# PKU-VCL-Geometry/GeoSplatting

Measured on AMD Instinct MI355X. Metric: fwd+bwd views/sec at 2M Gaussians, 800x800, higher is better.
Workload: dtype f32

## Files before the change

geosplatting_amd/csrc/gs_cube.h:

```cpp
#pragma once
#include "gs_common.h"

struct FaceMap { int a, b, c; float sx, sy; };
__device__ __forceinline__ FaceMap face_map(int s)
{
    const int axis = s >> 1;
    FaceMap m;
    m.a = axis == 0 ? 2 : 0;
    m.b = axis == 1 ? 2 : 1;
    m.c = axis;
    m.sx = (s == 0 || s == 5) ? -1.0f : 1.0f;
    m.sy = s == 2 ? 1.0f : -1.0f;
    return m;
}

__device__ __forceinline__ int select_face(const float* d)
{
    const float ax = fabsf(d[0]), ay = fabsf(d[1]), az = fabsf(d[2]);
    int f; float c;
    if (az > fmaxf(ax, ay)) { f = 4; c = d[2]; }
    else if (ay > ax)       { f = 2; c = d[1]; }
    else                    { f = 0; c = d[0]; }
    return f + (c < 0.0f ? 1 : 0);
}
// ... 102 lines not shown
    for (int i = 0; i < 4; ++i) { ok[i] = valid && fp.idx[i] >= 0; safe[i] = ok[i] ? fp.idx[i] : 0; }
    float t[4][3];
#pragma unroll
    for (int i = 0; i < 4; ++i) {
        const float* p = tex + (size_t)safe[i] * 3;
        t[i][0] = p[0]; t[i][1] = p[1]; t[i][2] = p[2];
    }
    bool has_miss = false;
#pragma unroll
    for (int i = 0; i < 4; ++i) {
        if (!ok[i]) { t[i][0] = t[i][1] = t[i][2] = 0.0f; }
        has_miss = has_miss || (valid && fp.idx[i] < 0);
    }
    if (has_miss) {
#pragma unroll
        for (int c = 0; c < 3; ++c) {
            const float s = (t[0][c] + t[1][c] + t[2][c] + t[3][c]) / 3.0f;
#pragma unroll
            for (int i = 0; i < 4; ++i) if (fp.idx[i] < 0) t[i][c] = s;
        }
    }
    if (!valid) {
        out[0] = out[1] = out[2] = 0.0f;
        if (WITH_GRAD) { for (int i = 0; i < 9; ++i) dd[i] = 0.0f; }
        return;
    }
    const FaceMap m = face_map(fp.face);
    const float sgn_c = comp3(d, m.c) < 0.0f ? -1.0f : 1.0f;
#pragma unroll
    for (int c = 0; c < 3; ++c) {
        const float top = t[0][c] + fp.fx * (t[1][c] - t[0][c]);
        const float bot = t[2][c] + fp.fx * (t[3][c] - t[2][c]);
        out[c] = top + fp.fy * (bot - top);
        if (WITH_GRAD) {
            const float dtx = (t[1][c] - t[0][c]) + fp.fy * ((t[3][c] - t[2][c]) - (t[1][c] - t[0][c]));
            const float dty = bot - top;
            const float gx = dtx * 0.5f * (float)R, gy = dty * 0.5f * (float)R;
            float g[3] = { 0.0f, 0.0f, 0.0f };
            const float va = gx * m.sx * fp.inv_c, vb = gy * m.sy * fp.inv_c;
            const float vc = -(gx * fp.xn + gy * fp.yn) * fp.inv_c * sgn_c;
#pragma unroll
            for (int k = 0; k < 3; ++k) g[k] = (k == m.a ? va : 0.0f) + (k == m.b ? vb : 0.0f) + (k == m.c ? vc : 0.0f);
            dd[c * 3 + 0] = g[0]; dd[c * 3 + 1] = g[1]; dd[c * 3 + 2] = g[2];
        }
    }
}

template <bool XCD_LOCAL>
__device__ __forceinline__ void gs_add_scoped(float* p, float v)
{
    if (XCD_LOCAL) gs_atomic_add_xcd(p, v); else gs_atomic_add(p, v);
}

template <bool XCD_LOCAL>
__device__ __forceinline__ void wave_commit6_lds(float* stage, float* pa, float* pb, const float (&v)[6])
{
    const int lane = (int)(threadIdx.x & 63);
    unsigned long long* sp = reinterpret_cast<unsigned long long*>(stage);
    float* sv = stage + 256;
    __builtin_amdgcn_wave_barrier();
    sp[lane] = (unsigned long long)pa; sp[64 + lane] = (unsigned long long)pb;
#pragma unroll
    for (int c = 0; c < 6; ++c) sv[c * 64 + lane] = v[c];
    __builtin_amdgcn_fence(__ATOMIC_RELEASE, "wavefront");
    __builtin_amdgcn_wave_barrier();
    __builtin_amdgcn_fence(__ATOMIC_ACQUIRE, "wavefront");
#pragma unroll
    for (int k = 0; k < 6; ++k) {
        const int q = 64 * k + lane;
        const int src = q / 6, ch = q - 6 * src;
        const bool second = ch >= 3;
        float* base = (float*)sp[(second ? 64 : 0) + src];
        const float val = sv[ch * 64 + src];
        if (base != nullptr) gs_add_scoped<XCD_LOCAL>(base + (second ? ch - 3 : ch), val);
    }
}

template <bool XCD_LOCAL>
__device__ __forceinline__ void wave_add6(float* pa, float* pb, const float (&v)[6], float* stage)
{
    float* enda = nullptr; float* endb = nullptr;
    float pv[6] = { 0.f, 0.f, 0.f, 0.f, 0.f, 0.f };
    if (pa != nullptr || pb != nullptr) {
        enda = pa; endb = pb;
#pragma unroll
        for (int c = 0; c < 6; ++c) pv[c] = v[c];
    }
    wave_commit6_lds<XCD_LOCAL>(stage, enda, endb, pv);
}

template <bool XCD_LOCAL>
__device__ __forceinline__ void cube_scatter_wave(float* grad_tex, const CubeFp& fp, const float* g, float scale, bool valid,
                                                  float* stage)
{
#pragma unroll
    for (int row = 0; row < 2; ++row) {
        float* p[2]; float v[6];
#pragma unroll
        for (int j = 0; j < 2; ++j) {
            const int i = 2 * row + j;
            const bool on = valid && fp.valid && fp.idx[i] >= 0 && grad_tex != nullptr;
            const float w = on ? scale * fp.w[i] : 0.0f;
            p[j] = on ? grad_tex + (size_t)fp.idx[i] * 3 : nullptr;
            v[3 * j] = g[0] * w; v[3 * j + 1] = g[1] * w; v[3 * j + 2] = g[2] * w;
        }
        wave_add6<XCD_LOCAL>(p[0], p[1], v, stage);
    }
}

__device__ __forceinline__ void wave_commit6_lds_tagged(float* stage, float* pa, float* pb, const float (&v)[6])
{
    const int lane = (int)(threadIdx.x & 63);
    unsigned long long* sp = reinterpret_cast<unsigned long long*>(stage);
    float* sv = stage + 256;
    const bool act = pa != nullptr || pb != nullptr;
    const unsigned long long am = __ballot(act);
    if (am == 0ull) return;
    const int n6 = 6 * __popcll(am);
    const int rank = __popcll(am & ((1ull << lane) - 1ull));
    __builtin_amdgcn_wave_barrier();
    if (act) {
        sp[rank] = (unsigned long long)pa; sp[64 + rank] = (unsigned long long)pb;
#pragma unroll
        for (int c = 0; c < 6; ++c) sv[c * 64 + rank] = v[c];
    }
    __builtin_amdgcn_fence(__ATOMIC_RELEASE, "wavefront");
    __builtin_amdgcn_wave_barrier();
    __builtin_amdgcn_fence(__ATOMIC_ACQUIRE, "wavefront");
    for (int k = 0; 64 * k < n6; ++k) {
        const int q = 64 * k + lane;
        if (q < n6) {
            const int src = q / 6, ch = q - 6 * src;
            const bool second = ch >= 3;
            const unsigned long long tagged = sp[(second ? 64 : 0) + src];
            float* base = (float*)(tagged & ~1ull);
            const float val = sv[ch * 64 + src];
            if (base != nullptr) {
                float* dst = base + (second ? ch - 3 : ch);
                if (tagged & 1ull) gs_atomic_add_xcd(dst, val); else gs_atomic_add(dst, val);
            }
        }
    }
}

__device__ __forceinline__ void cube_scatter_wave_tagged(float* grad_tex, bool local, const CubeFp& fp, const float* g, float scale, bool valid,
                                                         float* stage)
{
#pragma unroll
    for (int row = 0; row < 2; ++row) {
        float* p[2]; float v[6];
#pragma unroll
        for (int j = 0; j < 2; ++j) {
            const int i = 2 * row + j;
            const bool on = valid && fp.valid && fp.idx[i] >= 0 && grad_tex != nullptr;
            const float w = on ? scale * fp.w[i] : 0.0f;
            p[j] = on ? (float*)((unsigned long long)(grad_tex + (size_t)fp.idx[i] * 3) | (local ? 1ull : 0ull)) : nullptr;
            v[3 * j] = g[0] * w; v[3 * j + 1] = g[1] * w; v[3 * j + 2] = g[2] * w;
        }
        wave_commit6_lds_tagged(stage, p[0], p[1], v);
    }
}
```

geosplatting_amd/csrc/gs_front.hip:

```cpp
#include "gs_common.h"
#include <string.h>
#pragma clang fp contract(off)
#include "gs_project_dev.h"
#include "gs_shade_dev.h"

template <int CTRL, int ROW_MASK>
__device__ __forceinline__ unsigned dpp_max_u32(unsigned v)
{
    const unsigned o = (unsigned)__builtin_amdgcn_update_dpp(0, (int)v, CTRL, ROW_MASK, 0xf, false);
    return o > v ? o : v;
}
__device__ __forceinline__ unsigned wave_max_u32_lane63(unsigned v)
{
    v = dpp_max_u32<0xB1, 0xf>(v);
    v = dpp_max_u32<0x4E, 0xf>(v);
    v = dpp_max_u32<0x141, 0xf>(v);
    v = dpp_max_u32<0x140, 0xf>(v);
    v = dpp_max_u32<0x142, 0xa>(v);
    v = dpp_max_u32<0x143, 0xc>(v);
    return v;
}

#define GS_FRONT_BLOCK 256
#define GS_FRONT_ITEMS 2
// ... 465 lines not shown
    int W, H;
};
struct TailViewsDev { TailViewDev v[GS_TAIL_MAX_VIEWS]; int n; };

#define GS_TAILP_BLOCK 1024
struct TailViewLds {
    unsigned long long vis, v_packed, packed_index;
    float cam[16];
    float cam_pos[3];
    float Wf, Hf;
    float pad;
};

struct TailLevelLds { unsigned long long tex, gtex; long long priv_off; int R, lds_off; };

template <int VPG>
__device__ __forceinline__ float tail_group_sum(float v)
{
    if (VPG >= 2) v = gs_dpp_add<0xB1, 0xf, 0xf>(v);
    if (VPG >= 4) v = gs_dpp_add<0x4E, 0xf, 0xf>(v);
    if (VPG >= 8) v = gs_dpp_add<0x141, 0xf, 0xf>(v);
    return v;
}

template <int BLOCK, int VPG>
__global__ void __launch_bounds__(BLOCK)
tail_proj_pairs_kernel(int N, TailViewsDev views, const float* __restrict__ means, const float* __restrict__ quats,
                       const float* __restrict__ scales, const float* __restrict__ opacities, float eps2d, int rec_stride,
                       float* __restrict__ v_means, float* __restrict__ v_quats, float* __restrict__ v_scales,
                       float* __restrict__ v_opacities, int accumulate)
{
    __shared__ TailViewLds s_views[VPG];
#pragma unroll
    for (int k = 0; k < VPG; ++k) {
        if ((int)threadIdx.x == k) {
            const TailViewDev& h = views.v[k];
            TailViewLds& d = s_views[k];
            d.vis = (unsigned long long)h.vis; d.v_packed = (unsigned long long)h.v_packed; d.packed_index = (unsigned long long)h.packed_index;
            const GsCam c = load_cam(h.viewmat, h.K);
#pragma unroll
            for (int i = 0; i < 9; ++i) d.cam[i] = c.R[i];
            d.cam[9] = c.t[0]; d.cam[10] = c.t[1]; d.cam[11] = c.t[2];
            d.cam[12] = c.fx; d.cam[13] = c.fy; d.cam[14] = c.cx; d.cam[15] = c.cy;
            d.cam_pos[0] = d.cam_pos[1] = d.cam_pos[2] = 0.0f;
            d.Wf = (float)h.W; d.Hf = (float)h.H; d.pad = 0.0f;
        }
    }
    __syncthreads();
    constexpr int G = BLOCK / VPG;
    const int view = (int)threadIdx.x & (VPG - 1), gl = (int)threadIdx.x / VPG;
    const TailViewLds& vw = s_views[view];
    const int n = (int)blockIdx.x * G + gl;
    const bool live = n < N && view < views.n;
    const int slot = live ? reinterpret_cast<const int32_t*>(vw.packed_index)[n] : -1;
    ProjGrad pg;
#pragma unroll
    for (int c = 0; c < 3; ++c) { pg.mean[c] = 0.0f; pg.scale[c] = 0.0f; }
#pragma unroll
    for (int c = 0; c < 4; ++c) pg.quat[c] = 0.0f;
    pg.op = 0.0f;
    if (slot >= 0) {
        const float* vp = reinterpret_cast<const float*>(vw.v_packed) + (size_t)slot * rec_stride;
        const float4 g0 = reinterpret_cast<const float4*>(vp)[0];
        const float2 g1 = reinterpret_cast<const float2*>(vp)[2];
        if (g0.x != 0.0f || g0.y != 0.0f || g0.z != 0.0f || g0.w != 0.0f || g1.x != 0.0f || g1.y != 0.0f) {
            const float4* vis = reinterpret_cast<const float4*>(vw.vis);
            const float4 r0 = vis[4 * (size_t)slot], r1 = vis[4 * (size_t)slot + 1], r3 = vis[4 * (size_t)slot + 3];
            const float mean[3] = { means[3 * (size_t)n], means[3 * (size_t)n + 1], means[3 * (size_t)n + 2] };
            const float scale[3] = { scales[3 * (size_t)n], scales[3 * (size_t)n + 1], scales[3 * (size_t)n + 2] };
            const float4 q4 = *reinterpret_cast<const float4*>(quats + 4 * (size_t)n);
            const float opac = opacities[n];
            GsCam cam;
#pragma unroll
            for (int i = 0; i < 9; ++i) cam.R[i] = vw.cam[i];
            cam.t[0] = vw.cam[9]; cam.t[1] = vw.cam[10]; cam.t[2] = vw.cam[11];
            cam.fx = vw.cam[12]; cam.fy = vw.cam[13]; cam.cx = vw.cam[14]; cam.cy = vw.cam[15];
            project_bwd_one(cam, mean, q4, scale, opac, vw.Wf, vw.Hf, eps2d, 2.0f * r0.z, r0.w, 2.0f * r1.x, r3.x,
                            g0.x, g0.y, g0.z, g0.w, g1.x, g1.y, 0.0f, pg);
        }
    }
#pragma unroll
    for (int c = 0; c < 3; ++c) { pg.mean[c] = tail_group_sum<VPG>(pg.mean[c]); pg.scale[c] = tail_group_sum<VPG>(pg.scale[c]); }
#pragma unroll
    for (int c = 0; c < 4; ++c) pg.quat[c] = tail_group_sum<VPG>(pg.quat[c]);
    pg.op = tail_group_sum<VPG>(pg.op);
    if (n < N) {
        if (view == 0 % VPG) {
#pragma unroll
            for (int c = 0; c < 3; ++c) v_means[3 * (size_t)n + c] += pg.mean[c];
        }
        if (view == 1 % VPG) {
            float4 q = accumulate ? *reinterpret_cast<float4*>(v_quats + 4 * (size_t)n) : make_float4(0.f, 0.f, 0.f, 0.f);
            q.x += pg.quat[0]; q.y += pg.quat[1]; q.z += pg.quat[2]; q.w += pg.quat[3];
            *reinterpret_cast<float4*>(v_quats + 4 * (size_t)n) = q;
        }
        if (view == 2 % VPG) {
#pragma unroll
            for (int c = 0; c < 3; ++c) v_scales[3 * (size_t)n + c] = (accumulate ? v_scales[3 * (size_t)n + c] : 0.0f) + pg.scale[c];
        }
        if (view == 3 % VPG) v_opacities[n] = (accumulate ? v_opacities[n] : 0.0f) + pg.op;
    }
}

template <int BLOCK, int VPG, bool DIFFUSE>
__global__ void __launch_bounds__(BLOCK)
tail_shade_pairs_kernel(int N, TailViewsDev views, const float* __restrict__ means, const float* __restrict__ normals,
                        const float* __restrict__ kd, const float* __restrict__ ks, float min_roughness, float max_metallic, EnvDev env,
                        int rec_stride, float* __restrict__ v_means, float* __restrict__ v_normals, float* __restrict__ v_kd,
                        float* __restrict__ v_ks, EnvGradDev eg, int accumulate, int mode_rt)
{
    const int mode = DIFFUSE ? GS_MODE_DIFFUSE : mode_rt;
    __builtin_assume(DIFFUSE || mode != GS_MODE_DIFFUSE);
    extern __shared__ __attribute__((aligned(16))) float s_grad[];
    __shared__ TailViewLds s_views[VPG];
    __shared__ TailLevelLds s_levels[GS_MAX_LEVELS];
    for (int i = threadIdx.x; i < eg.lds_floats; i += blockDim.x) s_grad[i] = 0.0f;
#pragma unroll
    for (int l = 0; l < GS_MAX_LEVELS; ++l) {
        if ((int)threadIdx.x == 64 + l) {
            TailLevelLds& d = s_levels[l];
            if (DIFFUSE) { d.tex = (unsigned long long)env.base; d.gtex = (unsigned long long)eg.base; d.priv_off = -1; d.R = env.base_res; d.lds_off = eg.lds_base; }
            else { d.tex = (unsigned long long)env.levels[l]; d.gtex = (unsigned long long)eg.levels[l]; d.priv_off = eg.priv ? eg.priv_level[l] : -1; d.R = env.res[l]; d.lds_off = eg.lds_level[l]; }
        }
    }
#pragma unroll
    for (int k = 0; k < VPG; ++k) {
        if ((int)threadIdx.x == k) {
            const TailViewDev& h = views.v[k];
            TailViewLds& d = s_views[k];
            d.vis = (unsigned long long)h.vis; d.v_packed = (unsigned long long)h.v_packed; d.packed_index = (unsigned long long)h.packed_index;
            const GsCam c = load_cam(h.viewmat, h.K);
#pragma unroll
            for (int i = 0; i < 9; ++i) d.cam[i] = c.R[i];
            d.cam[9] = c.t[0]; d.cam[10] = c.t[1]; d.cam[11] = c.t[2];
            d.cam[12] = c.fx; d.cam[13] = c.fy; d.cam[14] = c.cx; d.cam[15] = c.cy;
            d.cam_pos[0] = h.cam_pos[0]; d.cam_pos[1] = h.cam_pos[1]; d.cam_pos[2] = h.cam_pos[2];
            d.Wf = (float)h.W; d.Hf = (float)h.H; d.pad = 0.0f;
        }
    }
    __syncthreads();
    float* const stage = s_grad + eg.stage_off + (threadIdx.x >> 6) * 640;
    float* const priv = eg.priv ? eg.priv + (long long)gs_xcc_id() * eg.priv_stride : nullptr;
    constexpr int G = BLOCK / VPG;
    const int view = (int)threadIdx.x & (VPG - 1), gl = (int)threadIdx.x / VPG;
    const bool view_on = view < views.n;
    const TailViewLds& vw = s_views[view];
    const int stride = (int)gridDim.x * G;
    const int n_iter = (N + stride - 1) / stride;
    for (int it = 0; it < n_iter; ++it) {
        const int n = it * stride + (int)blockIdx.x * G + gl;
        const bool live = n < N && view_on;
        const int slot = live ? reinterpret_cast<const int32_t*>(vw.packed_index)[n] : -1;
        float mean[3] = { 0, 0, 0 }, normal[3] = { 0, 0, 0 }, kdn[3] = { 0, 0, 0 }, ksn[2] = { 0, 0 };
        if (live) {
            mean[0] = means[3 * (size_t)n]; mean[1] = means[3 * (size_t)n + 1]; mean[2] = means[3 * (size_t)n + 2];
            normal[0] = normals[3 * (size_t)n]; normal[1] = normals[3 * (size_t)n + 1]; normal[2] = normals[3 * (size_t)n + 2];
            kdn[0] = kd[3 * (size_t)n]; kdn[1] = kd[3 * (size_t)n + 1]; kdn[2] = kd[3 * (size_t)n + 2];
            const float2 ks2 = *reinterpret_cast<const float2*>(ks + 2 * (size_t)n);
            ksn[0] = ks2.x; ksn[1] = ks2.y;
        }
        float a_mean[3] = { 0, 0, 0 }, a_n[3] = { 0, 0, 0 }, a_kd[3] = { 0, 0, 0 }, a_ks[2] = { 0, 0 };
        const float* vp = reinterpret_cast<const float*>(vw.v_packed) + (size_t)(slot >= 0 ? slot : 0) * rec_stride;
        bool work = false;
        PairPre pre;
        float g[3] = { 0, 0, 0 };
        if (slot >= 0) {
            g[0] = vp[6]; g[1] = vp[7]; g[2] = vp[8];
            if (g[0] != 0.0f || g[1] != 0.0f || g[2] != 0.0f) {
                const float cp[3] = { vw.cam_pos[0], vw.cam_pos[1], vw.cam_pos[2] };
                shade_pair_pre(mean, normal, kdn, ksn, cp, min_roughness, max_metallic, mode, env, g, pre);
                work = true;
            }
        }
        float o_acc[3] = { 0, 0, 0 }, vd_acc[3] = { 0, 0, 0 }, v_mip = 0.0f;
#pragma unroll 1
        for (int lv = 0; lv < (DIFFUSE ? 1 : 2); ++lv) {
            const int l = work ? (lv == 0 ? pre.l0 : pre.l1) : -1;
            const bool on = l >= 0;
            const TailLevelLds& lt = s_levels[on ? l : 0];
            const float w = lv == 0 ? (pre.l1 < 0 ? 1.0f : 1.0f - pre.f) : pre.f;
            CubeFp fp;
            fp.valid = false;
            if (on) {
                float o[3], sv, dd[3];
                cube_fetch_vjp(reinterpret_cast<const float*>(lt.tex), lt.R, pre.dir, pre.v, o, sv, dd, fp);
#pragma unroll
                for (int c = 0; c < 3; ++c) { o_acc[c] = fmaf(w, o[c], o_acc[c]); vd_acc[c] = fmaf(w, dd[c], vd_acc[c]); }
                v_mip += lv == 0 ? -sv : sv;
            }
            const bool in_lds = on && lt.lds_off >= 0;
            if (in_lds) cube_scatter_lds(s_grad + lt.lds_off, fp, pre.v, w);
            const bool glob = on && !in_lds;
            const bool loc = glob && priv != nullptr && lt.priv_off >= 0;
            cube_scatter_wave_tagged(glob ? (loc ? priv + lt.priv_off : reinterpret_cast<float*>(lt.gtex)) : nullptr, loc, fp, pre.v, w, glob, stage);
        }
        if (work) shade_pair_post(pre, normal, kdn, g, mode, min_roughness, max_metallic, o_acc, vd_acc, v_mip, a_mean, a_n, a_kd, a_ks);
#pragma unroll
        for (int c = 0; c < 3; ++c) {
            a_mean[c] = tail_group_sum<VPG>(a_mean[c]); a_n[c] = tail_group_sum<VPG>(a_n[c]); a_kd[c] = tail_group_sum<VPG>(a_kd[c]);
        }
        a_ks[0] = tail_group_sum<VPG>(a_ks[0]); a_ks[1] = tail_group_sum<VPG>(a_ks[1]);
        if (n < N) {
            if (view == 0 % VPG) {
#pragma unroll
                for (int c = 0; c < 3; ++c) v_means[3 * (size_t)n + c] = (accumulate ? v_means[3 * (size_t)n + c] : 0.0f) + a_mean[c];
            }
            if (view == 1 % VPG) {
                float2 o = accumulate ? *reinterpret_cast<float2*>(v_ks + 2 * (size_t)n) : make_float2(0.f, 0.f);
                o.x += a_ks[0]; o.y += a_ks[1];
                *reinterpret_cast<float2*>(v_ks + 2 * (size_t)n) = o;
            }
            if (view == 2 % VPG) {
#pragma unroll
                for (int c = 0; c < 3; ++c) v_normals[3 * (size_t)n + c] = (accumulate ? v_normals[3 * (size_t)n + c] : 0.0f) + a_n[c];
            }
            if (view == 3 % VPG) {
#pragma unroll
                for (int c = 0; c < 3; ++c) v_kd[3 * (size_t)n + c] = (accumulate ? v_kd[3 * (size_t)n + c] : 0.0f) + a_kd[c];
            }
        }
    }
    __syncthreads();
    if (eg.lds_base >= 0) {
        const int cnt = 18 * env.base_res * env.base_res;
        for (int i = threadIdx.x; i < cnt; i += blockDim.x) {
            const float x = s_grad[eg.lds_base + i];
            if (x != 0.0f) gs_atomic_add(eg.base + i, x);
        }
    }
    for (int l = 0; l < env.L; ++l) {
        if (eg.lds_level[l] < 0) continue;
        const int cnt = 18 * env.res[l] * env.res[l];
        for (int i = threadIdx.x; i < cnt; i += blockDim.x) {
            const float x = s_grad[eg.lds_level[l] + i];
            if (x != 0.0f) gs_atomic_add(eg.levels[l] + i, x);
        }
    }
}

extern "C" int gs_tail_bwd_multi_parts(int parts, int N, int n_views, const GsTailView* views, const float* means, const float* quats,
                                       const float* scales, const float* opacities, const float* normals, const float* kd, const float* ks,
                                       float min_roughness, float max_metallic, int mode, const GsEnv* env, float eps2d, int rec_stride,
                                       float* v_means, float* v_quats, float* v_scales, float* v_opacities, float* v_normals, float* v_kd,
                                       float* v_ks, int accumulate, const GsEnvGrad* env_grad, void* priv_ws, size_t priv_ws_bytes, void* stream)
{
    GS_CHECK_ARG(parts >= 1 && parts <= 7 && (parts & 3) != 0, "parts: bit 0 = shading backward, bit 1 = projection backward, bit 2 = background launch");
    GS_CHECK_ARG(N >= 0 && n_views >= 1 && mode >= 0 && mode <= 2 && rec_stride >= 12 && (rec_stride % 4) == 0, "bad sizes, mode or record stride");
    GS_CHECK_ARG(views != nullptr && env_grad != nullptr, "null argument");
    EnvDev e;
    GS_CHECK_ARG(env_to_dev(env, e) == 0, "bad GsEnv");
    EnvGradDev eg;
    { const int rc = env_grad_to_dev(__func__, env_grad, e, mode, eg); if (rc != GS_OK) return rc; }
    ShadeBwdPlan plan;
    { const int rc = shade_bwd_plan(e, mode, N, GS_TAILP_BLOCK, nullptr, 0, eg, plan); if (rc != GS_OK) return rc; }
    { const int rc = tail_priv_to_dev("gs_tail_bwd_multi", e, mode, priv_ws, priv_ws_bytes, eg); if (rc != GS_OK) return rc; }
    if (N == 0) return GS_OK;
    hipStream_t s = (hipStream_t)stream;
    for (int v0 = 0; v0 < n_views; v0 += GS_TAIL_MAX_VIEWS) {
        TailViewsDev tv;
        tv.n = (n_views - v0) < GS_TAIL_MAX_VIEWS ? (n_views - v0) : GS_TAIL_MAX_VIEWS;
        for (int k = 0; k < tv.n; ++k) {
            const GsTailView& h = views[v0 + k];
            GS_CHECK_ARG(h.viewmat && h.K && h.cam_pos && h.vis_records && h.v_packed && h.packed_index && h.W > 0 && h.H > 0, "bad GsTailView");
            tv.v[k] = TailViewDev{ h.viewmat, h.K, h.cam_pos, (const float4*)h.vis_records, h.v_packed, h.packed_index, h.W, h.H };
        }
        for (int k = tv.n; k < GS_TAIL_MAX_VIEWS; ++k) tv.v[k] = tv.v[0];
        const int acc = (accumulate || v0 > 0) ? 1 : 0;
#define GS_TAILP_LAUNCH(B, VPG, DIFF)                                                                                                    \
        do {                                                                                                                            \
            const int groups = gs_cdiv(N, B / VPG);                                                                                     \
            int max_blocks = eg.lds_floats > 0 ? 256 * (int)fmax(1.0, floor(160.0 * 1024.0 / (double)(plan.lds_bytes + 2048))) : 2048; \
// ... 112 lines not shown
```

geosplatting_amd/csrc/gs_shade_dev.h:

```cpp
#pragma once
#include "gs_common.h"
#include <stdlib.h>
#include <math.h>
#include "gs_cube.h"

struct EnvDev {
    const float* lut; int lut_res;
    const float* base; int base_res;
    int L;
    const float* levels[GS_MAX_LEVELS];
    int res[GS_MAX_LEVELS];
    float min_r, max_r;
};
struct EnvGradDev {
    float* base;
    float* levels[GS_MAX_LEVELS];
    int lds_base;
    int lds_level[GS_MAX_LEVELS];
    int lds_floats;
    int stage_off;
    float* priv;
    long long priv_stride;
    long long priv_level[GS_MAX_LEVELS];
    long long priv_base;
// ... 140 lines not shown
                                              float* v_ks, float* o_mean)
{
    float v_diff[3] = { 0, 0, 0 }, v_rf[3] = { 0, 0, 0 };
#pragma unroll
    for (int c = 0; c < 3; ++c) {
        if (mode == GS_MODE_PBR)          { v_diff[c] = g[c]; v_ls[c] = g[c] * t.refl_c[c]; v_rf[c] = g[c] * t.ls.out[c]; }
        else if (mode == GS_MODE_DIFFUSE) { v_ld[c] = g[c] * t.diff[c]; v_diff[c] = g[c] * t.ld[c]; }
        else                              { v_ls[c] = g[c] * t.refl_c[c]; v_rf[c] = g[c] * t.ls.out[c]; }
    }
    float v_A = 0.0f, v_B = 0.0f, v_metal = 0.0f;
#pragma unroll
    for (int c = 0; c < 3; ++c) {
        const float v_spec = v_rf[c] * t.fg[0];
        v_A += v_rf[c] * t.spec[c];
        v_B += v_rf[c];
        o_kd[c] = v_spec * t.metal + v_diff[c] * (1.0f - t.metal);
        v_metal += v_spec * (kd[c] - 0.04f) - v_diff[c] * kd[c];
    }
    const float v_ndv = v_A * t.dfg_du[0] + v_B * t.dfg_du[1];
    float v_rough = v_A * t.dfg_dv[0] + v_B * t.dfg_dv[1];
    float v_mip = 0.0f, v_refl[3] = { 0, 0, 0 };
    v_n[0] = v_n[1] = v_n[2] = 0.0f;
    if (mode != GS_MODE_DIFFUSE) {
#pragma unroll
        for (int c = 0; c < 3; ++c) {
            v_mip += v_ls[c] * t.ls.dmip[c];
#pragma unroll
            for (int k = 0; k < 3; ++k) v_refl[k] += v_ls[c] * t.ls.dd[c * 3 + k];
        }
    } else {
#pragma unroll
        for (int c = 0; c < 3; ++c)
#pragma unroll
            for (int k = 0; k < 3; ++k) v_n[k] += v_ld[c] * t.ld_dd[c * 3 + k];
    }
    v_rough += v_mip * t.dmip_dr;
    float v_d = 2.0f * (v_refl[0] * normal[0] + v_refl[1] * normal[1] + v_refl[2] * normal[2]);
    float v_wo[3];
#pragma unroll
    for (int k = 0; k < 3; ++k) { v_n[k] += 2.0f * t.d * v_refl[k]; v_wo[k] = -v_refl[k]; }
    if (t.d >= 1e-6f) v_d += v_ndv;
#pragma unroll
    for (int k = 0; k < 3; ++k) { v_n[k] += v_d * t.wo[k]; v_wo[k] += v_d * normal[k]; }
    o_mean[0] = o_mean[1] = o_mean[2] = 0.0f;
    if (!t.wo_const) {
        const float dot = t.wo[0] * v_wo[0] + t.wo[1] * v_wo[1] + t.wo[2] * v_wo[2];
        const float l = fmaxf(t.len, 1e-6f);
#pragma unroll
        for (int k = 0; k < 3; ++k) o_mean[k] = -((v_wo[k] - t.wo[k] * dot) / l);
    }
    v_ks[0] = v_rough * (1.0f - min_roughness); v_ks[1] = v_metal * max_metallic;
}

__device__ __forceinline__ void cube_fetch_vjp(const float* __restrict__ tex, int R, const float* d, const float* v, float* out,
                                               float& s, float* v_d, CubeFp& fp)
{
    cube_footprint(d, R, fp);
    const bool valid = fp.valid;
    bool ok[4]; int safe[4];
#pragma unroll
    for (int i = 0; i < 4; ++i) { ok[i] = valid && fp.idx[i] >= 0; safe[i] = ok[i] ? fp.idx[i] : 0; }
    float t[4][3];
#pragma unroll
    for (int i = 0; i < 4; ++i) {
        const float* p = tex + (size_t)safe[i] * 3;
        t[i][0] = p[0]; t[i][1] = p[1]; t[i][2] = p[2];
    }
    bool has_miss = false;
#pragma unroll
    for (int i = 0; i < 4; ++i) {
        if (!ok[i]) { t[i][0] = t[i][1] = t[i][2] = 0.0f; }
        has_miss = has_miss || (valid && fp.idx[i] < 0);
    }
    if (has_miss) {
#pragma unroll
        for (int c = 0; c < 3; ++c) {
            const float m = (t[0][c] + t[1][c] + t[2][c] + t[3][c]) / 3.0f;
#pragma unroll
            for (int i = 0; i < 4; ++i) if (fp.idx[i] < 0) t[i][c] = m;
        }
    }
    {
#pragma clang fp contract(fast)
        float q[4];
#pragma unroll
        for (int i = 0; i < 4; ++i) q[i] = v[0] * t[i][0] + v[1] * t[i][1] + v[2] * t[i][2];
#pragma unroll
        for (int c = 0; c < 3; ++c) {
            const float top = t[0][c] + fp.fx * (t[1][c] - t[0][c]);
            const float bot = t[2][c] + fp.fx * (t[3][c] - t[2][c]);
            out[c] = valid ? top + fp.fy * (bot - top) : 0.0f;
        }
        const float qt = q[0] + fp.fx * (q[1] - q[0]), qb = q[2] + fp.fx * (q[3] - q[2]);
        s = valid ? qt + fp.fy * (qb - qt) : 0.0f;
        const float dtx = (q[1] - q[0]) + fp.fy * ((q[3] - q[2]) - (q[1] - q[0]));
        const float dty = qb - qt;
        const FaceMap m = face_map(fp.face);
        const float sgn_c = comp3(d, m.c) < 0.0f ? -1.0f : 1.0f;
        const float gx = dtx * 0.5f * (float)R, gy = dty * 0.5f * (float)R;
        const float va = gx * m.sx * fp.inv_c, vb = gy * m.sy * fp.inv_c;
        const float vc = -(gx * fp.xn + gy * fp.yn) * fp.inv_c * sgn_c;
#pragma unroll
        for (int k = 0; k < 3; ++k) v_d[k] = valid ? (k == m.a ? va : 0.0f) + (k == m.b ? vb : 0.0f) + (k == m.c ? vc : 0.0f) : 0.0f;
    }
}

struct PairPre {
    float metal, spec[3], wo[3], len, d;
    float fg0, dfg_du[2], dfg_dv[2];
    float dir[3];
    float v[3];
    float dmip_dr, f;
    int l0, l1;
    bool wo_const, clamped;
};

__device__ __forceinline__ void shade_pair_pre(const float* mean, const float* normal, const float* kd, const float* ks, const float* cam_pos,
                                               float min_roughness, float max_metallic, int mode, const EnvDev& env, const float* g, PairPre& p)
{
    const float rough = ks[0] * (1.0f - min_roughness) + min_roughness;
    p.metal = ks[1] * max_metallic;
    const float vv[3] = { cam_pos[0] - mean[0], cam_pos[1] - mean[1], cam_pos[2] - mean[2] };
    p.len = sqrtf(vv[0] * vv[0] + vv[1] * vv[1] + vv[2] * vv[2]);
    if (p.len < 1e-6f) { p.wo[0] = 0.0f; p.wo[1] = 0.0f; p.wo[2] = 1.0f; p.wo_const = true; }
    else { const float l = fmaxf(p.len, 1e-6f); p.wo[0] = vv[0] / l; p.wo[1] = vv[1] / l; p.wo[2] = vv[2] / l; p.wo_const = false; }
    p.d = normal[0] * p.wo[0] + normal[1] * p.wo[1] + normal[2] * p.wo[2];
    const float ndv = fmaxf(p.d, 1e-6f);
    float fg[2];
    tex2d_linear_clamp2(env.lut, env.lut_res, env.lut_res, ndv, rough, fg, p.dfg_du, p.dfg_dv);
    p.fg0 = fg[0];
    const float mip = mip_from_roughness(rough, env.min_r, env.max_r, env.L, p.dmip_dr);
    const int L = env.L;
    const float lam = fminf(fmaxf(mip, 0.0f), (float)(L - 1));
    const int lf = (int)floorf(lam);
    const bool last = lf >= L - 1;
    p.l0 = last ? L - 1 : lf;
    p.l1 = last ? -1 : lf + 1;
    p.f = last ? 0.0f : lam - (float)p.l0;
    p.clamped = last || (mip < 0.0f || mip > (float)(L - 1));
#pragma unroll
    for (int c = 0; c < 3; ++c) p.spec[c] = (1.0f - p.metal) * 0.04f + kd[c] * p.metal;
    if (mode != GS_MODE_DIFFUSE) {
#pragma unroll
        for (int k = 0; k < 3; ++k) { p.dir[k] = 2.0f * p.d * normal[k] - p.wo[k]; p.v[k] = g[k] * (p.spec[k] * fg[0] + fg[1]); }
    } else {
#pragma unroll
        for (int k = 0; k < 3; ++k) { p.dir[k] = normal[k]; p.v[k] = g[k] * (kd[k] * (1.0f - p.metal)); }
        p.l0 = 0; p.l1 = -1; p.f = 0.0f;
    }
}

__device__ __forceinline__ void shade_pair_post(const PairPre& p, const float* normal, const float* kd, const float* g, int mode,
                                                float min_roughness, float max_metallic, const float* o, const float* v_dir, float v_mip,
                                                float* a_mean, float* a_n, float* a_kd, float* a_ks)
{
#pragma clang fp contract(fast)
    float v_diff[3] = { 0, 0, 0 }, v_rf[3] = { 0, 0, 0 }, v_refl[3] = { 0, 0, 0 }, v_n[3] = { 0, 0, 0 };
#pragma unroll
    for (int c = 0; c < 3; ++c) {
        if (mode == GS_MODE_DIFFUSE) { v_diff[c] = g[c] * o[c]; v_n[c] = v_dir[c]; }
        else { v_rf[c] = g[c] * o[c]; v_refl[c] = v_dir[c]; if (mode == GS_MODE_PBR) v_diff[c] = g[c]; }
    }
    float v_A = 0.0f, v_B = 0.0f, v_metal = 0.0f;
#pragma unroll
    for (int c = 0; c < 3; ++c) {
        const float v_spec = v_rf[c] * p.fg0;
        v_A += v_rf[c] * p.spec[c];
        v_B += v_rf[c];
        a_kd[c] += v_spec * p.metal + v_diff[c] * (1.0f - p.metal);
        v_metal += v_spec * (kd[c] - 0.04f) - v_diff[c] * kd[c];
    }
    const float v_ndv = v_A * p.dfg_du[0] + v_B * p.dfg_du[1];
    const float v_rough = v_A * p.dfg_dv[0] + v_B * p.dfg_dv[1] + ((p.clamped || mode == GS_MODE_DIFFUSE) ? 0.0f : v_mip) * p.dmip_dr;
    float v_d = 2.0f * (v_refl[0] * normal[0] + v_refl[1] * normal[1] + v_refl[2] * normal[2]);
    float v_wo[3];
#pragma unroll
    for (int j = 0; j < 3; ++j) { v_n[j] += 2.0f * p.d * v_refl[j]; v_wo[j] = -v_refl[j]; }
    if (p.d >= 1e-6f) v_d += v_ndv;
#pragma unroll
    for (int j = 0; j < 3; ++j) { v_n[j] += v_d * p.wo[j]; v_wo[j] += v_d * normal[j]; }
    if (!p.wo_const) {
        const float dot = p.wo[0] * v_wo[0] + p.wo[1] * v_wo[1] + p.wo[2] * v_wo[2];
        const float rl = __builtin_amdgcn_rcpf(fmaxf(p.len, 1e-6f));
#pragma unroll
        for (int j = 0; j < 3; ++j) a_mean[j] -= (v_wo[j] - p.wo[j] * dot) * rl;
    }
#pragma unroll
    for (int j = 0; j < 3; ++j) a_n[j] += v_n[j];
    a_ks[0] += v_rough * (1.0f - min_roughness); a_ks[1] += v_metal * max_metallic;
}

__device__ __forceinline__ void cube_scatter_lds(float* lds, const CubeFp& fp, const float* g, float scale)
{
    if (!fp.valid) return;
#pragma unroll
    for (int i = 0; i < 4; ++i) {
        if (fp.idx[i] < 0) continue;
        const float w = scale * fp.w[i];
        float* p = lds + (size_t)fp.idx[i] * 3;
        atomicAdd(p, g[0] * w); atomicAdd(p + 1, g[1] * w); atomicAdd(p + 2, g[2] * w);
    }
}

struct CommitDevice {
    __device__ __forceinline__ void operator()(float* glob, long long, const CubeFp& fp, const float* v, float w, bool on, float* stage) const
    { cube_scatter_wave<false>(on ? glob : nullptr, fp, v, w, on, stage); }
};
struct CommitTagged {
    float* priv;
    __device__ __forceinline__ void operator()(float* glob, long long priv_off, const CubeFp& fp, const float* v, float w, bool on, float* stage) const
    {
        const bool loc = on && priv != nullptr && priv_off >= 0;
        cube_scatter_wave_tagged(on ? (loc ? priv + priv_off : glob) : nullptr, loc, fp, v, w, on, stage);
    }
};

template <class Commit>
__device__ __forceinline__ void env_scatter_wave(const EnvGradDev& eg, float* s_grad, float* stage, const Commit& commit, bool base, int l,
                                                 const CubeFp& fp, const float* v, float w)
{
// ... 120 lines not shown
```

Before: 764.5.

## Software-pipeline tail shading loads and defer cube gradient scatters

Restructures the per-Gaussian tail backward loop so the next iteration's per-Gaussian inputs, cotangent and slot index are prefetched with inline-asm global loads and waited on late. Texture gradient scatters to LDS and global memory are deferred until after the group reductions, and the old output values are read before the wait. The aim is to hide global memory latency behind the shading math. It also uses address-space-1 pointers for global loads and atomics, uses mbcnt for the lane rank, and recomputes the spec term instead of storing it in PairPre to reduce register pressure. Risks include hand-written waitcnt and asm correctness, higher register use from keeping the prefetch live, and extra LDS traffic for parking the first level's footprint.

```diff
diff --git a/geosplatting_amd/csrc/gs_cube.h b/geosplatting_amd/csrc/gs_cube.h
--- a/geosplatting_amd/csrc/gs_cube.h
+++ b/geosplatting_amd/csrc/gs_cube.h
@@ -178,6 +178,30 @@
     if (XCD_LOCAL) gs_atomic_add_xcd(p, v); else gs_atomic_add(p, v);
 }
 
+#define GS_GLOBAL __attribute__((address_space(1)))
+typedef float gs_gv2f __attribute__((ext_vector_type(2)));
+typedef float gs_gv3f __attribute__((ext_vector_type(3)));
+typedef float gs_gv4f __attribute__((ext_vector_type(4)));
+__device__ __forceinline__ GS_GLOBAL float* gs_global(unsigned long long a) { return (GS_GLOBAL float*)a; }
+__device__ __forceinline__ GS_GLOBAL const float* gs_global_c(unsigned long long a) { return (GS_GLOBAL const float*)a; }
+__device__ __forceinline__ float4 gs_gload4(GS_GLOBAL const float* p)
+{
+    const gs_gv4f v = *(GS_GLOBAL const gs_gv4f*)p;
+    return make_float4(v.x, v.y, v.z, v.w);
+}
+__device__ __forceinline__ float2 gs_gload2(GS_GLOBAL const float* p)
+{
+    const gs_gv2f v = *(GS_GLOBAL const gs_gv2f*)p;
+    return make_float2(v.x, v.y);
+}
+__device__ __forceinline__ void gs_atomic_add(GS_GLOBAL float* p, float v) { __hip_atomic_fetch_add(p, v, __ATOMIC_RELAXED, __HIP_MEMORY_SCOPE_AGENT); }
+__device__ __forceinline__ void gs_atomic_add_xcd(GS_GLOBAL float* p, float v) { __hip_atomic_fetch_add(p, v, __ATOMIC_RELAXED, __HIP_MEMORY_SCOPE_WORKGROUP); }
+template <bool XCD_LOCAL>
+__device__ __forceinline__ void gs_add_scoped(GS_GLOBAL float* p, float v)
+{
+    if (XCD_LOCAL) gs_atomic_add_xcd(p, v); else gs_atomic_add(p, v);
+}
+
 template <bool XCD_LOCAL>
 __device__ __forceinline__ void wave_commit6_lds(float* stage, float* pa, float* pb, const float (&v)[6])
 {
@@ -196,9 +220,9 @@
         const int q = 64 * k + lane;
         const int src = q / 6, ch = q - 6 * src;
         const bool second = ch >= 3;
-        float* base = (float*)sp[(second ? 64 : 0) + src];
+        const unsigned long long staged = sp[(second ? 64 : 0) + src];
         const float val = sv[ch * 64 + src];
-        if (base != nullptr) gs_add_scoped<XCD_LOCAL>(base + (second ? ch - 3 : ch), val);
+        if (staged != 0ull) gs_add_scoped<XCD_LOCAL>(gs_global(staged) + (second ? ch - 3 : ch), val);
     }
 }
 
@@ -243,7 +267,7 @@
     const unsigned long long am = __ballot(act);
     if (am == 0ull) return;
     const int n6 = 6 * __popcll(am);
-    const int rank = __popcll(am & ((1ull << lane) - 1ull));
+    const int rank = (int)__builtin_amdgcn_mbcnt_hi((unsigned)(am >> 32), __builtin_amdgcn_mbcnt_lo((unsigned)am, 0u));
     __builtin_amdgcn_wave_barrier();
     if (act) {
         sp[rank] = (unsigned long long)pa; sp[64 + rank] = (unsigned long long)pb;
@@ -259,10 +283,10 @@
             const int src = q / 6, ch = q - 6 * src;
             const bool second = ch >= 3;
             const unsigned long long tagged = sp[(second ? 64 : 0) + src];
-            float* base = (float*)(tagged & ~1ull);
+            const unsigned long long base = tagged & ~1ull;
             const float val = sv[ch * 64 + src];
-            if (base != nullptr) {
-                float* dst = base + (second ? ch - 3 : ch);
+            if (base != 0ull) {
+                GS_GLOBAL float* dst = gs_global(base) + (second ? ch - 3 : ch);
                 if (tagged & 1ull) gs_atomic_add_xcd(dst, val); else gs_atomic_add(dst, val);
             }
         }
diff --git a/geosplatting_amd/csrc/gs_front.hip b/geosplatting_amd/csrc/gs_front.hip
--- a/geosplatting_amd/csrc/gs_front.hip
+++ b/geosplatting_amd/csrc/gs_front.hip
@@ -541,7 +541,7 @@
     const TailViewLds& vw = s_views[view];
     const int n = (int)blockIdx.x * G + gl;
     const bool live = n < N && view < views.n;
-    const int slot = live ? reinterpret_cast<const int32_t*>(vw.packed_index)[n] : -1;
+    const int slot = live ? ((GS_GLOBAL const int32_t*)vw.packed_index)[n] : -1;
     ProjGrad pg;
 #pragma unroll
     for (int c = 0; c < 3; ++c) { pg.mean[c] = 0.0f; pg.scale[c] = 0.0f; }
@@ -549,12 +549,12 @@
     for (int c = 0; c < 4; ++c) pg.quat[c] = 0.0f;
     pg.op = 0.0f;
     if (slot >= 0) {
-        const float* vp = reinterpret_cast<const float*>(vw.v_packed) + (size_t)slot * rec_stride;
-        const float4 g0 = reinterpret_cast<const float4*>(vp)[0];
-        const float2 g1 = reinterpret_cast<const float2*>(vp)[2];
+        GS_GLOBAL const float* vp = gs_global_c(vw.v_packed) + (size_t)slot * rec_stride;
+        const float4 g0 = gs_gload4(vp);
+        const float2 g1 = gs_gload2(vp + 4);
         if (g0.x != 0.0f || g0.y != 0.0f || g0.z != 0.0f || g0.w != 0.0f || g1.x != 0.0f || g1.y != 0.0f) {
-            const float4* vis = reinterpret_cast<const float4*>(vw.vis);
-            const float4 r0 = vis[4 * (size_t)slot], r1 = vis[4 * (size_t)slot + 1], r3 = vis[4 * (size_t)slot + 3];
+            GS_GLOBAL const float* vis = gs_global_c(vw.vis) + 16 * (size_t)slot;
+            const float4 r0 = gs_gload4(vis), r1 = gs_gload4(vis + 4), r3 = gs_gload4(vis + 12);
             const float mean[3] = { means[3 * (size_t)n], means[3 * (size_t)n + 1], means[3 * (size_t)n + 2] };
             const float scale[3] = { scales[3 * (size_t)n], scales[3 * (size_t)n + 1], scales[3 * (size_t)n + 2] };
             const float4 q4 = *reinterpret_cast<const float4*>(quats + 4 * (size_t)n);
@@ -589,6 +589,30 @@
         }
         if (view == 3 % VPG) v_opacities[n] = (accumulate ? v_opacities[n] : 0.0f) + pg.op;
     }
+}
+
+__device__ __forceinline__ int tail_opaque_uniform(int x) { int y; asm volatile("s_mov_b32 %0, %1" : "=s"(y) : "s"(x)); return y; }
+__device__ __forceinline__ float tail_opaque_uniform(float x) { return __int_as_float(tail_opaque_uniform(__float_as_int(x))); }
+struct TailPrefetch { gs_gv3f mean, normal, kd, g; gs_gv2f ks; int slot; };
+__device__ __forceinline__ void tail_load(TailPrefetch& p, const float* means, const float* normals, const float* kd, const float* ks, unsigned r,
+                                          GS_GLOBAL const float* cot, GS_GLOBAL const int32_t* slot)
+{
+    const unsigned r12 = 12u * r, r8 = 8u * r;
+    asm volatile("global_load_dwordx3 %0, %1, off" : "=&v"(p.g) : "v"(cot) : "memory");
+    asm volatile("global_load_dword %0, %1, off" : "=&v"(p.slot) : "v"(slot) : "memory");
+    asm volatile("global_load_dwordx3 %0, %1, %2" : "=&v"(p.mean) : "v"(r12), "s"(means) : "memory");
+    asm volatile("global_load_dwordx3 %0, %1, %2" : "=&v"(p.normal) : "v"(r12), "s"(normals) : "memory");
+    asm volatile("global_load_dwordx3 %0, %1, %2" : "=&v"(p.kd) : "v"(r12), "s"(kd) : "memory");
+    asm volatile("global_load_dwordx2 %0, %1, %2" : "=&v"(p.ks) : "v"(r8), "s"(ks) : "memory");
+}
+__device__ __forceinline__ void tail_wait(TailPrefetch& p)
+{
+    __builtin_amdgcn_s_waitcnt(0x0F70);
+    asm volatile("" : : "v"(p.mean), "v"(p.normal), "v"(p.kd), "v"(p.g), "v"(p.ks), "v"(p.slot) : "memory");
+}
+__device__ __forceinline__ void tail_take(TailPrefetch& p)
+{
+    asm volatile("" : "+v"(p.mean), "+v"(p.normal), "+v"(p.kd), "+v"(p.g), "+v"(p.ks), "+v"(p.slot) : : "memory");
 }
 
 template <int BLOCK, int VPG, bool DIFFUSE>
@@ -636,76 +660,128 @@
     const TailViewLds& vw = s_views[view];
     const int stride = (int)gridDim.x * G;
     const int n_iter = (N + stride - 1) / stride;
+    const int n_first = (int)blockIdx.x * G + gl;
+    const auto row = [&](int it) -> size_t { const long long r = (long long)it * stride + n_first; return (size_t)(r < N ? r : N - 1); };
+    const auto cot_ptr = [&](int slot) -> GS_GLOBAL const float* {
+        return slot >= 0 ? gs_global_c(vw.v_packed) + (size_t)slot * rec_stride + 6 : (GS_GLOBAL const float*)means;
+    };
+    TailPrefetch pf;
+    int slot_raw = ((GS_GLOBAL const int32_t*)vw.packed_index)[row(0)];
+    tail_load(pf, means, normals, kd, ks, (unsigned)row(0), cot_ptr(slot_raw), (GS_GLOBAL const int32_t*)vw.packed_index + row(1));
+    tail_wait(pf);
     for (int it = 0; it < n_iter; ++it) {
-        const int n = it * stride + (int)blockIdx.x * G + gl;
+        tail_take(pf);
+        EnvDev envi = env;
+        envi.L = tail_opaque_uniform(env.L); envi.lut_res = tail_opaque_uniform(env.lut_res);
+        envi.min_r = tail_opaque_uniform(env.min_r); envi.max_r = tail_opaque_uniform(env.max_r);
+        const float min_rough = tail_opaque_uniform(min_roughness), max_metal = tail_opaque_uniform(max_metallic);
+        const int n = it * stride + n_first;
         const bool live = n < N && view_on;
-        const int slot = live ? reinterpret_cast<const int32_t*>(vw.packed_index)[n] : -1;
-        float mean[3] = { 0, 0, 0 }, normal[3] = { 0, 0, 0 }, kdn[3] = { 0, 0, 0 }, ksn[2] = { 0, 0 };
-        if (live) {
-            mean[0] = means[3 * (size_t)n]; mean[1] = means[3 * (size_t)n + 1]; mean[2] = means[3 * (size_t)n + 2];
-            normal[0] = normals[3 * (size_t)n]; normal[1] = normals[3 * (size_t)n + 1]; normal[2] = normals[3 * (size_t)n + 2];
-            kdn[0] = kd[3 * (size_t)n]; kdn[1] = kd[3 * (size_t)n + 1]; kdn[2] = kd[3 * (size_t)n + 2];
-            const float2 ks2 = *reinterpret_cast<const float2*>(ks + 2 * (size_t)n);
-            ksn[0] = ks2.x; ksn[1] = ks2.y;
-        }
+        const int slot = live ? slot_raw : -1;
+        const float mean[3] = { pf.mean.x, pf.mean.y, pf.mean.z }, normal[3] = { pf.normal.x, pf.normal.y, pf.normal.z };
+        const float kdn[3] = { pf.kd.x, pf.kd.y, pf.kd.z }, ksn[2] = { pf.ks.x, pf.ks.y };
+        const float g[3] = { pf.g.x, pf.g.y, pf.g.z };
         float a_mean[3] = { 0, 0, 0 }, a_n[3] = { 0, 0, 0 }, a_kd[3] = { 0, 0, 0 }, a_ks[2] = { 0, 0 };
-        const float* vp = reinterpret_cast<const float*>(vw.v_packed) + (size_t)(slot >= 0 ? slot : 0) * rec_stride;
         bool work = false;
         PairPre pre;
-        float g[3] = { 0, 0, 0 };
-        if (slot >= 0) {
-            g[0] = vp[6]; g[1] = vp[7]; g[2] = vp[8];
-            if (g[0] != 0.0f || g[1] != 0.0f || g[2] != 0.0f) {
-                const float cp[3] = { vw.cam_pos[0], vw.cam_pos[1], vw.cam_pos[2] };
-                shade_pair_pre(mean, normal, kdn, ksn, cp, min_roughness, max_metallic, mode, env, g, pre);
-                work = true;
-            }
-        }
+        if (slot >= 0 && (g[0] != 0.0f || g[1] != 0.0f || g[2] != 0.0f)) {
+            const float cp[3] = { vw.cam_pos[0], vw.cam_pos[1], vw.cam_pos[2] };
+            shade_pair_pre(mean, normal, kdn, ksn, cp, min_rough, max_metal, mode, envi, g, pre);
+            work = true;
+        }
+        const bool any = __ballot(work) != 0ull;
+        const int l0 = work ? pre.l0 : -1, l1 = (!DIFFUSE && work) ? pre.l1 : -1;
+        const bool on0 = l0 >= 0, on1 = l1 >= 0;
+        const float w0 = on1 ? 1.0f - pre.f : 1.0f, w1 = on1 ? pre.f : 0.0f;
         float o_acc[3] = { 0, 0, 0 }, vd_acc[3] = { 0, 0, 0 }, v_mip = 0.0f;
+        CubeFp fp0, fp1;
+        fp0.valid = false; fp1.valid = false;
+        if (any) {
 #pragma unroll 1
-        for (int lv = 0; lv < (DIFFUSE ? 1 : 2); ++lv) {
-            const int l = work ? (lv == 0 ? pre.l0 : pre.l1) : -1;
-            const bool on = l >= 0;
-            const TailLevelLds& lt = s_levels[on ? l : 0];
-            const float w = lv == 0 ? (pre.l1 < 0 ? 1.0f : 1.0f - pre.f) : pre.f;
-            CubeFp fp;
-            fp.valid = false;
-            if (on) {
-                float o[3], sv, dd[3];
-                cube_fetch_vjp(reinterpret_cast<const float*>(lt.tex), lt.R, pre.dir, pre.v, o, sv, dd, fp);
-#pragma unroll
-                for (int c = 0; c < 3; ++c) { o_acc[c] = fmaf(w, o[c], o_acc[c]); vd_acc[c] = fmaf(w, dd[c], vd_acc[c]); }
-                v_mip += lv == 0 ? -sv : sv;
-            }
-            const bool in_lds = on && lt.lds_off >= 0;
-            if (in_lds) cube_scatter_lds(s_grad + lt.lds_off, fp, pre.v, w);
-            const bool glob = on && !in_lds;
-            const bool loc = glob && priv != nullptr && lt.priv_off >= 0;
-            cube_scatter_wave_tagged(glob ? (loc ? priv + lt.priv_off : reinterpret_cast<float*>(lt.gtex)) : nullptr, loc, fp, pre.v, w, glob, stage);
-        }
-        if (work) shade_pair_post(pre, normal, kdn, g, mode, min_roughness, max_metallic, o_acc, vd_acc, v_mip, a_mean, a_n, a_kd, a_ks);
+            for (int lv = 0; lv < (DIFFUSE ? 1 : 2); ++lv) {
+                const int l = lv == 0 ? l0 : l1;
+                CubeFp fp;
+                fp.valid = false;
+                if (l >= 0) {
+                    const TailLevelLds& lt = s_levels[l];
+                    const float w = lv == 0 ? w0 : w1;
+                    float o[3], sv, dd[3];
+                    cube_fetch_vjp(gs_global_c(lt.tex), lt.R, pre.dir, pre.v, o, sv, dd, fp);
+#pragma unroll
+                    for (int c = 0; c < 3; ++c) { o_acc[c] = fmaf(w, o[c], o_acc[c]); vd_acc[c] = fmaf(w, dd[c], vd_acc[c]); }
+                    v_mip += lv == 0 ? -sv : sv;
+                }
+                if (!DIFFUSE && lv == 0) {
+                    float4* const park = reinterpret_cast<float4*>(stage) + 2 * (threadIdx.x & 63);
+                    park[0] = make_float4(__int_as_float(fp.idx[0]), __int_as_float(fp.idx[1]), __int_as_float(fp.idx[2]), __int_as_float(fp.idx[3]));
+                    park[1] = make_float4(fp.w[0], fp.w[1], fp.w[2], fp.w[3]);
+                    fp0.valid = fp.valid;
+                } else {
+                    fp1 = fp;
+                }
+            }
+        }
+        if (work) shade_pair_post(pre, normal, kdn, g, mode, min_rough, max_metal, o_acc, vd_acc, v_mip, a_mean, a_n, a_kd, a_ks);
 #pragma unroll
         for (int c = 0; c < 3; ++c) {
             a_mean[c] = tail_group_sum<VPG>(a_mean[c]); a_n[c] = tail_group_sum<VPG>(a_n[c]); a_kd[c] = tail_group_sum<VPG>(a_kd[c]);
         }
         a_ks[0] = tail_group_sum<VPG>(a_ks[0]); a_ks[1] = tail_group_sum<VPG>(a_ks[1]);
+        slot_raw = pf.slot;
+        {
+            const long long u = (long long)(it + 1) * stride;
+            const size_t ub = (size_t)(u < N ? u : N - 1);
+            tail_load(pf, means + 3 * ub, normals + 3 * ub, kd + 3 * ub, ks + 2 * ub, (unsigned)(row(it + 1) - ub), cot_ptr(slot_raw),
+                      (GS_GLOBAL const int32_t*)vw.packed_index + row(it + 2));
+        }
+        constexpr int OWN = VPG >= 4 ? 1 : 4 / VPG;
+        float b_old[OWN][3];
+#pragma unroll
+        for (int j = 0; j < OWN; ++j) {
+            const int k = view + j * VPG;
+            const size_t r = row(it);
+            const float* p = k == 1 ? v_ks + 2 * r : (k == 2 ? v_normals + 3 * r : (k == 3 ? v_kd + 3 * r : v_means + 3 * r));
+            b_old[j][0] = b_old[j][1] = b_old[j][2] = 0.0f;
+            if (accumulate) { b_old[j][0] = p[0]; b_old[j][1] = p[1]; b_old[j][2] = p[k == 1 ? 0 : 2]; }
+        }
+        if (any) {
+            if (!DIFFUSE) {
+                const float4* const park = reinterpret_cast<const float4*>(stage) + 2 * (threadIdx.x & 63);
+                const float4 pi = park[0], pw = park[1];
+                fp0.idx[0] = __float_as_int(pi.x); fp0.idx[1] = __float_as_int(pi.y); fp0.idx[2] = __float_as_int(pi.z); fp0.idx[3] = __float_as_int(pi.w);
+                fp0.w[0] = pw.x; fp0.w[1] = pw.y; fp0.w[2] = pw.z; fp0.w[3] = pw.w;
+            }
+            if (on0 && s_levels[l0].lds_off >= 0) cube_scatter_lds(s_grad + s_levels[l0].lds_off, DIFFUSE ? fp1 : fp0, pre.v, w0);
+            if (!DIFFUSE && on1 && s_levels[l1].lds_off >= 0) cube_scatter_lds(s_grad + s_levels[l1].lds_off, fp1, pre.v, w1);
+        }
+        tail_wait(pf);
         if (n < N) {
             if (view == 0 % VPG) {
 #pragma unroll
-                for (int c = 0; c < 3; ++c) v_means[3 * (size_t)n + c] = (accumulate ? v_means[3 * (size_t)n + c] : 0.0f) + a_mean[c];
+                for (int c = 0; c < 3; ++c) v_means[3 * (size_t)n + c] = b_old[0 / VPG % OWN][c] + a_mean[c];
             }
             if (view == 1 % VPG) {
-                float2 o = accumulate ? *reinterpret_cast<float2*>(v_ks + 2 * (size_t)n) : make_float2(0.f, 0.f);
-                o.x += a_ks[0]; o.y += a_ks[1];
-                *reinterpret_cast<float2*>(v_ks + 2 * (size_t)n) = o;
+                const float* b = b_old[1 / VPG % OWN];
+                *reinterpret_cast<float2*>(v_ks + 2 * (size_t)n) = make_float2(b[0] + a_ks[0], b[1] + a_ks[1]);
             }
             if (view == 2 % VPG) {
 #pragma unroll
-                for (int c = 0; c < 3; ++c) v_normals[3 * (size_t)n + c] = (accumulate ? v_normals[3 * (size_t)n + c] : 0.0f) + a_n[c];
+                for (int c = 0; c < 3; ++c) v_normals[3 * (size_t)n + c] = b_old[2 / VPG % OWN][c] + a_n[c];
             }
             if (view == 3 % VPG) {
 #pragma unroll
-                for (int c = 0; c < 3; ++c) v_kd[3 * (size_t)n + c] = (accumulate ? v_kd[3 * (size_t)n + c] : 0.0f) + a_kd[c];
+                for (int c = 0; c < 3; ++c) v_kd[3 * (size_t)n + c] = b_old[3 / VPG % OWN][c] + a_kd[c];
+            }
+        }
+        if (any) {
+#pragma unroll
+            for (int lv = 0; lv < (DIFFUSE ? 1 : 2); ++lv) {
+                const bool on = lv == 0 ? on0 : on1;
+                const TailLevelLds& lt = s_levels[on ? (lv == 0 ? l0 : l1) : 0];
+                const bool glob = on && lt.lds_off < 0;
+                const bool loc = glob && priv != nullptr && lt.priv_off >= 0;
+                cube_scatter_wave_tagged(glob ? (loc ? priv + lt.priv_off : reinterpret_cast<float*>(lt.gtex)) : nullptr, loc, (!DIFFUSE && lv == 0) ? fp0 : fp1,
+                                         pre.v, lv == 0 ? w0 : w1, glob, stage);
             }
         }
     }
diff --git a/geosplatting_amd/csrc/gs_shade_dev.h b/geosplatting_amd/csrc/gs_shade_dev.h
--- a/geosplatting_amd/csrc/gs_shade_dev.h
+++ b/geosplatting_amd/csrc/gs_shade_dev.h
@@ -216,24 +216,27 @@
     v_ks[0] = v_rough * (1.0f - min_roughness); v_ks[1] = v_metal * max_metallic;
 }
 
-__device__ __forceinline__ void cube_fetch_vjp(const float* __restrict__ tex, int R, const float* d, const float* v, float* out,
-                                               float& s, float* v_d, CubeFp& fp)
-{
-    cube_footprint(d, R, fp);
+struct CubeTaps { float t[4][3]; };
+template <class Tex>
+__device__ __forceinline__ void cube_taps_issue(Tex __restrict__ tex, const CubeFp& fp, CubeTaps& x)
+{
+#pragma unroll
+    for (int i = 0; i < 4; ++i) {
+        const int safe = (fp.valid && fp.idx[i] >= 0) ? fp.idx[i] : 0;
+        const Tex p = tex + (size_t)safe * 3;
+        x.t[i][0] = p[0]; x.t[i][1] = p[1]; x.t[i][2] = p[2];
+    }
+}
+
+__device__ __forceinline__ void cube_taps_vjp(CubeTaps& x, int R, const float* d, const float* v, const CubeFp& fp, float* out,
+                                              float& s, float* v_d)
+{
+    float (&t)[4][3] = x.t;
     const bool valid = fp.valid;
-    bool ok[4]; int safe[4];
-#pragma unroll
-    for (int i = 0; i < 4; ++i) { ok[i] = valid && fp.idx[i] >= 0; safe[i] = ok[i] ? fp.idx[i] : 0; }
-    float t[4][3];
+    bool has_miss = false;
 #pragma unroll
     for (int i = 0; i < 4; ++i) {
-        const float* p = tex + (size_t)safe[i] * 3;
-        t[i][0] = p[0]; t[i][1] = p[1]; t[i][2] = p[2];
-    }
-    bool has_miss = false;
-#pragma unroll
-    for (int i = 0; i < 4; ++i) {
-        if (!ok[i]) { t[i][0] = t[i][1] = t[i][2] = 0.0f; }
+        if (!(valid && fp.idx[i] >= 0)) { t[i][0] = t[i][1] = t[i][2] = 0.0f; }
         has_miss = has_miss || (valid && fp.idx[i] < 0);
     }
     if (has_miss) {
@@ -269,8 +272,24 @@
     }
 }
 
+template <class Tex>
+__device__ __forceinline__ void cube_fetch_vjp(Tex __restrict__ tex, int R, const float* d, const float* v, float* out,
+                                               float& s, float* v_d, CubeFp& fp)
+{
+    cube_footprint(d, R, fp);
+    CubeTaps x;
+    cube_taps_issue(tex, fp, x);
+    cube_taps_vjp(x, R, d, v, fp, out, s, v_d);
+}
+
+__device__ __forceinline__ float pair_spec(float metal, float kd)
+{
+#pragma clang fp contract(off)
+    return (1.0f - metal) * 0.04f + kd * metal;
+}
+
 struct PairPre {
-    float metal, spec[3], wo[3], len, d;
+    float metal, wo[3], len, d;
     float fg0, dfg_du[2], dfg_dv[2];
     float dir[3];
     float v[3];
@@ -302,11 +321,9 @@
     p.l1 = last ? -1 : lf + 1;
     p.f = last ? 0.0f : lam - (float)p.l0;
     p.clamped = last || (mip < 0.0f || mip > (float)(L - 1));
-#pragma unroll
-    for (int c = 0; c < 3; ++c) p.spec[c] = (1.0f - p.metal) * 0.04f + kd[c] * p.metal;
     if (mode != GS_MODE_DIFFUSE) {
 #pragma unroll
-        for (int k = 0; k < 3; ++k) { p.dir[k] = 2.0f * p.d * normal[k] - p.wo[k]; p.v[k] = g[k] * (p.spec[k] * fg[0] + fg[1]); }
+        for (int k = 0; k < 3; ++k) { p.dir[k] = 2.0f * p.d * normal[k] - p.wo[k]; p.v[k] = g[k] * (pair_spec(p.metal, kd[k]) * fg[0] + fg[1]); }
     } else {
 #pragma unroll
         for (int k = 0; k < 3; ++k) { p.dir[k] = normal[k]; p.v[k] = g[k] * (kd[k] * (1.0f - p.metal)); }
@@ -329,7 +346,7 @@
 #pragma unroll
     for (int c = 0; c < 3; ++c) {
         const float v_spec = v_rf[c] * p.fg0;
-        v_A += v_rf[c] * p.spec[c];
+        v_A += v_rf[c] * pair_spec(p.metal, kd[c]);
         v_B += v_rf[c];
         a_kd[c] += v_spec * p.metal + v_diff[c] * (1.0f - p.metal);
         v_metal += v_spec * (kd[c] - 0.04f) - v_diff[c] * kd[c];
```

New measurement: 762.3. No clear change (-0.3%).
